# lightkurve/lightkurve

Measured on AMD Instinct MI355X. Metric: frequencies*targets/sec (Lomb-Scargle, ls_method='fast' (reference default): extirpolation + FFT) + BLS periods*targets/sec; max-power rel-err, higher is better.
Workload: dtype f64

## Files before the change

lightkurve_amd/csrc/lsfast.hip:

```cpp
#include <cmath>
#include <cstdlib>
#include <type_traits>
#include <vector>

#include "lk_common.hpp"
#include "ls_epilogue.hpp"

namespace lk {

typedef double lk_d2v __attribute__((ext_vector_type(2)));

constexpr int SPREAD_W = 1024;
constexpr int SPREAD_WW = 256;

struct FastStats {
    double wsum, ybar, YY, t0;
    double yws;
    double wmax;
    double vmax;
};

__device__ __forceinline__ void cadence_weights(const double *__restrict__ y, const double *__restrict__ dy, int64_t i,
                                                double wsum, double ybar, double &w, double &wy) {
    const double d = dy ? dy[i] : 1.0;
// ... 77 lines not shown
        }
        yws = bsum(acc2);
        wmx = bmax(wmx);
        vmx = bmax(vmx);
    }
    if (tid == 0) stats[b] = FastStats{wsum, ybar, YY, t0, yws, wmx, vmx};
}

constexpr int TAB_PER_LANE = 8;
__global__ __launch_bounds__(256) void lsf_tables_kernel(const double *__restrict__ t, const int64_t *__restrict__ n_off,
                                                          const FastStats *__restrict__ stats,
                                                          const int *__restrict__ rows_used, double df, int nfft, int m2,
                                                          int logW, int *__restrict__ spread_tab, int ntab) {
    const int b = blockIdx.y;
    if (!rows_used[b * 4 + 3]) return;
    const int64_t lo = n_off[b], n = n_off[b + 1] - lo;
    const int lane = threadIdx.x & 63;
    const int64_t base = ((int64_t)blockIdx.x * 4 + (threadIdx.x >> 6)) * (64 * TAB_PER_LANE);
    if (base >= n) return;
    const double t0 = stats[b].t0;
    int *tab = spread_tab + (size_t)b * 4 * ntab;
    const double iW = 1.0 / (double)(1 << logW), dn = (double)nfft;
    auto posn = [&](double tt) {
        const double x = (tt - t0) * dn * df;
        return x < dn ? x : fmod(x, dn);
    };
    double p1[TAB_PER_LANE];
#pragma unroll
    for (int u = 0; u < TAB_PER_LANE; ++u) {
        const int64_t i = base + 64 * u + lane;
        p1[u] = posn(t[lo + (i < n ? i : n - 1)]);
    }
    const int nf0 = min(ntab, (int)((((long long)rows_used[b * 4 + 0] << m2) >> logW) + 3));
    const int nf2 = min(ntab, (int)((((long long)rows_used[b * 4 + 2] << m2) >> logW) + 3));
    double prev_last = base > 0 ? posn(t[lo + base - 1]) : -1e300;
#pragma unroll
    for (int u = 0; u < TAB_PER_LANE; ++u) {
        const int64_t i = base + 64 * u + lane;
        double pp1 = __shfl_up(p1[u], 1);
        if (lane == 0) pp1 = prev_last;
        prev_last = __shfl(p1[u], 63);
        if (i >= n) continue;
#pragma unroll
        for (int gg = 0; gg < 2; ++gg) {
            const double p = gg ? 2.0 * p1[u] : p1[u], pp = i > 0 ? (gg ? 2.0 * pp1 : pp1) : -1e300;
            int *lo_a = tab + (size_t)(2 * gg) * ntab, *hi_a = lo_a + ntab;
            const int nfill = gg ? nf2 : nf0;
            int k0 = i > 0 ? (int)floor((pp + 4.0) * iW) + 1 : 0, k1 = (int)floor((p + 4.0) * iW);
            for (int k = max(k0, 0); k <= min(k1, ntab - 1); ++k) lo_a[k] = (int)i;
            if (i == n - 1)
                for (int k = max(k1 + 1, 0); k < nfill; ++k) lo_a[k] = (int)n;
            k0 = i > 0 ? (int)floor((pp - 3.0) * iW) + 1 : 0;
            k1 = (int)floor((p - 3.0) * iW);
            for (int k = max(k0, 0); k <= min(k1, ntab - 1); ++k) hi_a[k] = (int)i;
            if (i == n - 1)
                for (int k = max(k1 + 1, 0); k < nfill; ++k) hi_a[k] = (int)n;
        }
    }
}

__device__ __forceinline__ void phase_factor(double f, double tt, double &c, double &s) {
    const double p = f * tt, e = fma(f, tt, -p);
    const double r = (p - rint(p)) + e;
    sincospi(2.0 * r, &s, &c);
}

struct Stencil4 {
    int i0, n;
    double wt[4];
};
__device__ __forceinline__ Stencil4 stencil4(double x, int nfft) {
    Stencil4 st;
    if (x == floor(x)) {
        st.i0 = (int)x;
        st.n = 1;
        st.wt[0] = 1.0;
        st.wt[1] = st.wt[2] = st.wt[3] = 0.0;
        return st;
    }
    int ilo = (int)(x - 2.0);
    ilo = min(max(ilo, 0), nfft - 4);
    const double d0 = x - (double)ilo, d1 = d0 - 1.0, d2 = d0 - 2.0, d3 = d0 - 3.0;
    st.i0 = ilo;
    st.n = 4;
    st.wt[3] = ((d0 * d1) * d2) * (1.0 / 6.0);
    st.wt[2] = ((d0 * d1) * d3) * -0.5;
    st.wt[1] = ((d0 * d2) * d3) * 0.5;
    st.wt[0] = ((d1 * d2) * d3) * (-1.0 / 6.0);
    return st;
}

struct Quantum {
    double q, iq;
    __device__ __forceinline__ void add(double *cell, double v) const {
        if (q > 0.0)
            atomicAdd(reinterpret_cast<unsigned long long *>(cell), (unsigned long long)(long long)rint(v * iq));
        else
            unsafeAtomicAdd(cell, v);
    }
};
__device__ __forceinline__ Quantum make_quantum(double vmax) {
    const double q = (vmax > 0.0 && isfinite(vmax)) ? ldexp(1.0, ilogb(1.25 * vmax) - 49) : 0.0;
    return Quantum{q, q > 0.0 ? 1.0 / q : 0.0};
}

__device__ __forceinline__ void extirpolate4(double2 *__restrict__ grid, const Stencil4 &sp, double hr, double hi,
                                             const Quantum &Q) {
#pragma unroll
    for (int k = 0; k < 4; ++k)
        if (k < sp.n) {
            Q.add(&grid[sp.i0 + k].x, hr * sp.wt[k]);
            Q.add(&grid[sp.i0 + k].y, hi * sp.wt[k]);
        }
}

__global__ __launch_bounds__(256) void lsf_scatter_kernel(const double *__restrict__ t, const double *__restrict__ y,
                                                           const double *__restrict__ dy,
                                                           const int64_t *__restrict__ n_off,
                                                           const FastStats *__restrict__ stats, int b0, double f0,
                                                           double df, int nfft, int fit_mean,
                                                           double2 *__restrict__ grids,
                                                           const int *__restrict__ rows_used) {
    if (rows_used && rows_used[blockIdx.y * 4 + 3]) return;
    const int b = b0 + blockIdx.y;
    const int64_t lo = n_off[b];
    const int n = (int)(n_off[b + 1] - lo);
    const int i = blockIdx.x * 256 + threadIdx.x;
    if (i >= n) return;
    const FastStats st = stats[b];
    const double tt = t[lo + i] - st.t0;
    double2 *g0 = grids + (size_t)blockIdx.y * 3 * nfft, *g1 = g0 + nfft, *g2 = g1 + nfft;
    double wi, wyi;
    cadence_weights(y, dy, lo + i, st.wsum, st.ybar, wi, wyi);
    const Quantum Qy = make_quantum(st.vmax), Qw = make_quantum(st.wmax);
    for (int fac = 1; fac <= 2; ++fac) {
        const double dff = df * (double)fac, f0f = f0 * (double)fac;
        double c = 1.0, s = 0.0;
        if (f0f > 0.0) phase_factor(f0f, tt, c, s);
        const Stencil4 sp = stencil4(fmod(tt * (double)nfft * dff, (double)nfft), nfft);
        if (fac == 1) {
            extirpolate4(g0, sp, wyi * c, wyi * s, Qy);
            if (fit_mean) extirpolate4(g1, sp, wi * c, wi * s, Qw);
        } else {
            extirpolate4(g2, sp, wi * c, wi * s, Qw);
        }
    }
}

__global__ __launch_bounds__(256) void lsf_spread_owner_kernel(const double *__restrict__ t, const double *__restrict__ y,
                                                                const double *__restrict__ dy,
                                                                const int64_t *__restrict__ n_off,
                                                                const FastStats *__restrict__ stats, int b0, double f0,
                                                                double df, int nfft, int m2, int fit_mean,
                                                                double2 *__restrict__ grids,
                                                                const int *__restrict__ rows_used,
                                                                const int *__restrict__ spread_tab, int ntab) {
    __shared__ double2 acc0[SPREAD_W], acc1[SPREAD_W];
    const int lb = blockIdx.y, tid = threadIdx.x;
    const bool pair = blockIdx.z == 0;
    if (!rows_used[lb * 4 + 3]) return;
    const int g = pair ? 0 : 2;
    const int ncell = rows_used[lb * 4 + g] << m2;
    const int c_lo = blockIdx.x * SPREAD_W, c_hi = min(c_lo + SPREAD_W, ncell);
    if (c_lo >= ncell) return;
    double2 *G0 = grids + ((size_t)lb * 3 + g) * (size_t)nfft, *G1 = G0 + nfft;
    const int b = b0 + lb;
    const int64_t lo = n_off[b];
    const FastStats st = stats[b];
    const double fac = pair ? 1.0 : 2.0;
    const double dff = df * fac, f0f = f0 * fac;
    for (int c = tid; c < SPREAD_W; c += 256) {
        acc0[c] = make_double2(0.0, 0.0);
        acc1[c] = make_double2(0.0, 0.0);
    }
    __syncthreads();
    const int lane = tid & 63, wv = tid >> 6;
    const int w_lo = c_lo + wv * SPREAD_WW, w_hi = min(w_lo + SPREAD_WW, c_hi);
    if (w_lo < w_hi) {
        const int *tab = spread_tab + ((size_t)b * 4 + (pair ? 0 : 2)) * ntab;
        const int kblk = blockIdx.x * (SPREAD_W / SPREAD_WW) + wv;
        const int i_lo = tab[kblk], i_hi = tab[ntab + min(kblk + 1, ntab - 1)];
        for (int i = i_lo + lane; i < i_hi; i += 64) {
            const double tt = t[lo + i] - st.t0;
            double wi, wyi;
            cadence_weights(y, dy, lo + i, st.wsum, st.ybar, wi, wyi);
            double c = 1.0, s = 0.0;
            if (f0f > 0.0) phase_factor(f0f, tt, c, s);
            const Stencil4 sp = stencil4(fmod(tt * (double)nfft * dff, (double)nfft), nfft);
            const double ar = (pair ? wyi : wi) * c, ai = (pair ? wyi : wi) * s, br = wi * c, bi = wi * s;
#pragma unroll
            for (int k = 0; k < 4; ++k) {
                const int cell = sp.i0 + k;
                if (k < sp.n && cell >= w_lo && cell < w_hi) {
                    unsafeAtomicAdd(&acc0[cell - c_lo].x, ar * sp.wt[k]);
                    unsafeAtomicAdd(&acc0[cell - c_lo].y, ai * sp.wt[k]);
                    if (pair && fit_mean) {
                        unsafeAtomicAdd(&acc1[cell - c_lo].x, br * sp.wt[k]);
                        unsafeAtomicAdd(&acc1[cell - c_lo].y, bi * sp.wt[k]);
                    }
                }
            }
        }
    }
    __syncthreads();
    for (int c = c_lo + tid; c < c_hi; c += 256) {
        G0[c] = acc0[c - c_lo];
        if (pair) G1[c] = acc1[c - c_lo];
    }
}

__device__ __forceinline__ void lds_fft_dit(double2 *x, const double2 *tw, int n, int m, int nf) {
    const int tid = threadIdx.x, nt = blockDim.x;
    const int halfn = n >> 1;
    for (int s = 1; s <= m; ++s) {
        const int half = 1 << (s - 1);
        const int tstep = n >> s;
        for (int p = tid; p < nf * halfn; p += nt) {
            const int f = p >> (m - 1), j = p & (halfn - 1);
            const int grp = j >> (s - 1), k = j & (half - 1);
            const int i0 = f * n + (grp << s) + k, i1 = i0 + half;
            const double2 wv = tw[k * tstep];
            const double2 a = x[i0], bq = x[i1];
            const double tr = wv.x * bq.x - wv.y * bq.y, ti = wv.x * bq.y + wv.y * bq.x;
            x[i0] = make_double2(a.x + tr, a.y + ti);
            x[i1] = make_double2(a.x - tr, a.y - ti);
        }
        __syncthreads();
    }
}

__device__ __forceinline__ void lds_twiddles(double2 *tw, int n) {
    for (int k = threadIdx.x; k < (n >> 1); k += blockDim.x) {
        double s, c;
        sincospi(2.0 * (double)k / (double)n, &s, &c);
        tw[k] = make_double2(c, s);
    }
}

__global__ __launch_bounds__(256) void fft_cols_kernel(double2 *__restrict__ grids, int m1, int m2, int CT) {
    extern __shared__ __attribute__((aligned(16))) double2 lds2[];
    const int N1 = 1 << m1, N2 = 1 << m2;
    double2 *x = lds2, *tw = lds2 + (size_t)CT * N1;
    double2 *G = grids + ((size_t)blockIdx.y << (m1 + m2));
    const int c0 = blockIdx.x * CT;
    lds_twiddles(tw, N1);
    for (int e = threadIdx.x; e < CT * N1; e += 256) {
        const int r = e / CT, cc = e - r * CT;
        const int rr = (int)(__brev((unsigned)r) >> (32 - m1));
        x[cc * N1 + rr] = G[(size_t)r * N2 + c0 + cc];
    }
    __syncthreads();
    lds_fft_dit(x, tw, N1, m1, CT);
    const double invN = 1.0 / (double)((size_t)1 << (m1 + m2));
    for (int e = threadIdx.x; e < CT * N1; e += 256) {
        const int k1 = e / CT, cc = e - k1 * CT;
        const long long ck = (long long)(c0 + cc) * k1;
        double s, c;
        sincospi(2.0 * (double)ck * invN, &s, &c);
        const double2 v = x[cc * N1 + k1];
        G[(size_t)k1 * N2 + c0 + cc] = make_double2(v.x * c - v.y * s, v.x * s + v.y * c);
    }
}

__global__ __launch_bounds__(256) void fft_rows_kernel(const double2 *__restrict__ grids, int m1, int m2, int RT,
                                                        int nkeep, double2 *__restrict__ spec) {
    extern __shared__ __attribute__((aligned(16))) double2 lds2[];
    const int N2 = 1 << m2;
    double2 *x = lds2, *tw = lds2 + (size_t)RT * N2;
    const double2 *G = grids + ((size_t)blockIdx.y << (m1 + m2));
    double2 *S = spec + (size_t)blockIdx.y * nkeep;
    const int r0 = blockIdx.x * RT;
    lds_twiddles(tw, N2);
    for (int e = threadIdx.x; e < RT * N2; e += 256) {
        const int rr = e / N2, c = e - rr * N2;
        const int cr = m2 ? (int)(__brev((unsigned)c) >> (32 - m2)) : 0;
        x[rr * N2 + cr] = G[(size_t)(r0 + rr) * N2 + c];
    }
    __syncthreads();
    lds_fft_dit(x, tw, N2, m2, RT);
    for (int e = threadIdx.x; e < RT * N2; e += 256) {
        const int k2 = e / RT, rr = e - k2 * RT;
        const long long k = (long long)(r0 + rr) + ((long long)k2 << m1);
        if (k < nkeep) S[k] = x[rr * N2 + k2];
    }
}

__device__ constexpr double R32C[16] = {1.0, 0.98078528040323043, 0.92387953251128674, 0.83146961230254524,
                                        0.70710678118654752, 0.55557023301960218, 0.38268343236508978,
                                        0.19509032201612825, 0.0, -0.19509032201612825, -0.38268343236508978,
                                        -0.55557023301960218, -0.70710678118654752, -0.83146961230254524,
                                        -0.92387953251128674, -0.98078528040323043};
__device__ constexpr double R32S[16] = {0.0, 0.19509032201612825, 0.38268343236508978, 0.55557023301960218,
                                        0.70710678118654752, 0.83146961230254524, 0.92387953251128674,
                                        0.98078528040323043, 1.0, 0.98078528040323043, 0.92387953251128674,
                                        0.83146961230254524, 0.70710678118654752, 0.55557023301960218,
                                        0.38268343236508978, 0.19509032201612825};

__host__ __device__ constexpr int brev_c(int x, int bits) {
    int r = 0;
    for (int i = 0; i < bits; ++i) r |= ((x >> i) & 1) << (bits - 1 - i);
    return r;
}

template <int L>
__device__ __forceinline__ void reg_fft(double2 (&v)[1 << L]) {
#pragma unroll
    for (int s = L; s >= 1; --s) {
        const int half = 1 << (s - 1);
#pragma unroll
        for (int g = 0; g < (1 << L); g += (1 << s)) {
#pragma unroll
            for (int k = 0; k < half; ++k) {
                const double2 a = v[g + k], b = v[g + k + half];
                v[g + k] = make_double2(a.x + b.x, a.y + b.y);
                const double dx = a.x - b.x, dy = a.y - b.y;
                const int ti = k * (32 >> s);
                if (ti == 0)
                    v[g + k + half] = make_double2(dx, dy);
                else if (ti == 8)
                    v[g + k + half] = make_double2(-dy, dx);
                else
                    v[g + k + half] = make_double2(dx * R32C[ti] - dy * R32S[ti], dx * R32S[ti] + dy * R32C[ti]);
            }
        }
    }
}

__device__ __forceinline__ double2 cmul(double2 a, double2 b) {
    return make_double2(a.x * b.x - a.y * b.y, a.x * b.y + a.y * b.x);
}

template <int LA, int LB, int MODE, class Load, class Store>
__device__ __forceinline__ void block_fft(int NF, double2 *tile, Load load, Store store, int tw = 1) {
    constexpr int A = 1 << LA, Bq = 1 << LB, n = A * Bq, LDT = Bq + 1, FST = A * LDT + 1;
    const int tid = threadIdx.x;
    if (tid < NF * Bq) {
        int f, j;
        if (MODE == 1) {
            f = tid % NF;
            j = tid / NF;
        } else if (MODE == 2) {
            const int jl = tid % tw, rest = tid / tw;
            f = rest % NF;
            j = jl + tw * (rest / NF);
        } else {
            f = tid / Bq;
            j = tid % Bq;
        }
        double2 v[A];
#pragma unroll
        for (int i = 0; i < A; ++i) v[i] = load(f, i * Bq + j);
        reg_fft<LA>(v);
        double s1, c1;
        sincospi(2.0 * (double)j / (double)n, &s1, &c1);
        const double2 step = make_double2(c1, s1);
        double2 w = make_double2(1.0, 0.0);
        double2 *row = tile + (size_t)f * FST + j;
#pragma unroll
        for (int ka = 0; ka < A; ++ka) {
            row[ka * LDT] = cmul(v[brev_c(ka, LA)], w);
            w = cmul(w, step);
        }
    }
    __syncthreads();
    if (tid < NF * A) {
        const int ka = tid / NF, f = tid - ka * NF;
        const double2 *row = tile + (size_t)f * FST + (size_t)ka * LDT;
        double2 u[Bq];
#pragma unroll
        for (int j = 0; j < Bq; ++j) u[j] = row[j];
        reg_fft<LB>(u);
#pragma unroll
        for (int kb = 0; kb < Bq; ++kb) store(f, ka + A * kb, u[brev_c(kb, LB)], kb);
    }
}

template <int LA, int LB>
__global__ __launch_bounds__(256) void fft_cols_reg_kernel(double2 *__restrict__ grids, int m2, int CT,
                                                            const int *__restrict__ rows_used,
                                                            double2 *__restrict__ gout, int tw) {
    extern __shared__ __attribute__((aligned(16))) double2 lds2[];
    constexpr int m1 = LA + LB, A = 1 << LA;
    const int N2 = 1 << m2;
    double2 *G = grids + ((size_t)blockIdx.y << (m1 + m2));
    const int c0 = blockIdx.x * CT;
    const int ru = rows_used ? rows_used[(blockIdx.y / 3) * 4 + (blockIdx.y % 3)] : (1 << m1);
    const double invN = 1.0 / (double)((size_t)1 << (m1 + m2));
    auto load = [&](int f, int r) -> double2 {
        return r < ru ? G[(size_t)r * N2 + c0 + f] : make_double2(0.0, 0.0);
    };
    int last_f = -1;
    double2 w = make_double2(1.0, 0.0), step = w;
    const int twl = 31 - __clz(max(tw, 1));
    auto store = [&](int f, int k1, double2 v, int) {
        const int c = c0 + f;
        if (f != last_f) {
            double s, cc;
            sincospi(2.0 * (double)((long long)c * k1) * invN, &s, &cc);
            w = make_double2(cc, s);
            sincospi(2.0 * (double)((long long)c * A) * invN, &s, &cc);
            step = make_double2(cc, s);
            last_f = f;
        }
        if (gout)
            gout[((size_t)blockIdx.y << (m1 + m2)) + ((((size_t)(c >> twl) << m1) + k1) << twl) + (c & (tw - 1))] = cmul(v, w);
        else
            G[(size_t)k1 * N2 + c] = cmul(v, w);
        w = cmul(w, step);
    };
    block_fft<LA, LB, 1>(CT, lds2, load, store);
}

constexpr int PRUNED_CT = 16;

constexpr int LSF_CHUNK_HALF_GB = 3;

template <int LP>
__global__ __launch_bounds__(PRUNED_CT * (1 << ((LP + 1) / 2)), 2) void fft_cols_pruned_kernel(
    const double2 *__restrict__ grids, int m1, int m2, const int *__restrict__ rows_used, double2 *__restrict__ gout,
    const double *__restrict__ t, const double *__restrict__ y, const double *__restrict__ dy,
    const int64_t *__restrict__ n_off, const FastStats *__restrict__ stats, int b0, double f0, double df, int fit_mean,
    const int *__restrict__ tab16, int ntab16) {
    extern __shared__ __attribute__((aligned(16))) double2 lds2[];
    constexpr int LA = (LP + 1) / 2, LB = LP / 2, A = 1 << LA, Bq = 1 << LB, P = 1 << LP, LDT = Bq + 1, FST = A * LDT + 1;
    constexpr int CT = PRUNED_CT, NT = CT * A;
    const int N1 = 1 << m1, N2 = 1 << m2, Q = N1 >> LP;
    const double2 *G = grids + ((size_t)blockIdx.y << (m1 + m2));
    const size_t tstride = (size_t)CT << m1, gstride = (size_t)(N2 / CT) * tstride;
    double2 *O = gout + (size_t)blockIdx.y * gstride + (size_t)blockIdx.x * tstride;
    const int c0 = blockIdx.x * CT;
    const int lbt = blockIdx.y / 3, g = blockIdx.y % 3;
    const int ru = rows_used[lbt * 4 + g];
    const int tid = threadIdx.x;
    const int f = tid % CT, jk = tid / CT;
    const bool p1 = jk < Bq, p2 = jk < A;
    const double invN1 = 1.0 / (double)N1, invN = 1.0 / (double)((size_t)1 << (m1 + m2));
    double2 xin[A];
    if (tab16 != nullptr && rows_used[lbt * 4 + 3]) {
        double2 *acc = lds2;
        for (int e = tid; e < ru * CT; e += NT) acc[e] = make_double2(0.0, 0.0);
        __syncthreads();
        if (!(g == 1 && !fit_mean)) {
            const int b = b0 + lbt;
            const int64_t lo = n_off[b];
            const FastStats st = stats[b];
            const double fac = g == 2 ? 2.0 : 1.0, dff = df * fac, f0f = f0 * fac, dn = (double)((size_t)1 << (m1 + m2));
            const int nfft = 1 << (m1 + m2);
            const int *tlo = tab16 + ((size_t)b * 4 + (g == 2 ? 2 : 0)) * ntab16, *thi = tlo + ntab16;
            const int S = g == 2 ? 4 : 8, rpi = 64 / S;
            const int lane = tid & 63, wv = tid >> 6, rr = lane / S, k = lane - rr * S;
            const int rpw = (ru + NT / 64 - 1) / (NT / 64);
            const int r_end = min(ru, (wv + 1) * rpw);
            auto visit = [&](int r, double ti, double yi, double di) {
                const double tt = ti - st.t0;
                const double wi = (1.0 / (di * di)) / st.wsum, wyi = wi * (yi - st.ybar);
                double c = 1.0, sn = 0.0;
                if (f0f > 0.0) phase_factor(f0f, tt, c, sn);
                const double xp = tt * dn * dff;
                const Stencil4 sp = stencil4(xp < dn ? xp : fmod(xp, dn), nfft);
                const double amp = g == 0 ? wyi : wi, ar = amp * c, ai = amp * sn;
                const int cbase = (r << m2) + c0;
#pragma unroll
                for (int q = 0; q < 4; ++q) {
                    const unsigned col = (unsigned)(sp.i0 + q - cbase);
                    if (q < sp.n && col < (unsigned)CT) {
                        unsafeAtomicAdd(&acc[r * CT + col].x, ar * sp.wt[q]);
                        unsafeAtomicAdd(&acc[r * CT + col].y, ai * sp.wt[q]);
                    }
                }
            };
            constexpr int UN = 4;
            for (int rb = wv * rpw; rb < r_end; rb += UN * rpi) {
                int ii[UN], ih[UN];
#pragma unroll
                for (int u = 0; u < UN; ++u) {
                    const int r = rb + u * rpi + rr;
                    const int blk = (min(r, r_end - 1) << (m2 - 4)) + blockIdx.x;
                    ii[u] = tlo[blk] + k;
                    ih[u] = thi[blk + 1];
                }
#pragma unroll
                for (int u = 0; u < UN; ++u) {
                    asm volatile("" : "+v"(ii[u]), "+v"(ih[u]));
                    if (rb + u * rpi + rr >= r_end) ii[u] = ih[u] = 0;
                }
                double tv[UN], yv[UN], dv[UN];
#pragma unroll
                for (int u = 0; u < UN; ++u) {
                    const bool ok = ii[u] < ih[u];
                    const int64_t ix = lo + (ok ? ii[u] : 0);
                    tv[u] = t[ix];
                    yv[u] = y[ix];
                    dv[u] = dy ? dy[ix] : 1.0;
                }
#pragma unroll
                for (int u = 0; u < UN; ++u) {
                    const int r = rb + u * rpi + rr;
                    if (ii[u] < ih[u]) visit(r, tv[u], yv[u], dv[u]);
                    int i = ii[u] + S;
                    while (__any(i < ih[u])) {
                        if (i < ih[u]) visit(r, t[lo + i], y[lo + i], dy ? dy[lo + i] : 1.0);
                        i += S;
                    }
                }
            }
        }
        __syncthreads();
        if (p1) {
#pragma unroll
            for (int i = 0; i < A; ++i) {
                const int r = i * Bq + jk;
                xin[i] = r < ru ? acc[r * CT + f] : make_double2(0.0, 0.0);
            }
        }
        __syncthreads();
    } else if (p1) {
#pragma unroll
        for (int i = 0; i < A; ++i) {
            const int r = i * Bq + jk;
            xin[i] = r < ru ? G[(size_t)r * N2 + c0 + f] : make_double2(0.0, 0.0);
        }
    }
    auto root = [](double x) {
        double sn, cs;
        sincospi(2.0 * x, &sn, &cs);
        return make_double2(cs, sn);
    };
    const double2 wj = root((double)jk * invN1), wq = root((double)Bq * invN1);
    const double2 tw_j = root((double)jk / (double)P);
    const double2 wc = root((double)(c0 + f) * invN), stepc = root((double)((long long)(c0 + f) * Q * A) * invN);
    double2 wjs = make_double2(1.0, 0.0), wqs = wjs;
    double2 wout = root((double)((long long)(c0 + f) * Q * jk) * invN);
    for (int s = 0; s < Q; ++s) {
        if (p1) {
            double2 v[A];
            if (s == 0) {
#pragma unroll
                for (int i = 0; i < A; ++i) v[i] = xin[i];
            } else {
                double2 w = wjs;
#pragma unroll
                for (int i = 0; i < A; ++i) {
                    v[i] = cmul(xin[i], w);
                    w = cmul(w, wqs);
                }
            }
            reg_fft<LA>(v);
            double2 w = make_double2(1.0, 0.0);
            double2 *row = lds2 + (size_t)f * FST + jk;
#pragma unroll
            for (int ka = 0; ka < A; ++ka) {
                row[ka * LDT] = cmul(v[brev_c(ka, LA)], w);
                w = cmul(w, tw_j);
            }
        }
        __syncthreads();
        if (p2) {
            const double2 *row = lds2 + (size_t)f * FST + (size_t)jk * LDT;
            double2 u[Bq];
#pragma unroll
            for (int j = 0; j < Bq; ++j) u[j] = row[j];
            reg_fft<LB>(u);
            double2 w = wout;
#pragma unroll
            for (int kb = 0; kb < Bq; ++kb) {
                const int q = jk + A * kb;
                O[(size_t)(Q * q + s) * CT + f] = cmul(u[brev_c(kb, LB)], w);
                w = cmul(w, stepc);
            }
        }
        wjs = cmul(wjs, wj);
        wqs = cmul(wqs, wq);
        wout = cmul(wout, wc);
        __syncthreads();
    }
}

template <int LA, int LB>
__global__ __launch_bounds__(256) void fft_rows_reg_kernel(const double2 *__restrict__ grids, int m1, int RT, int nkeep,
                                                            double2 *__restrict__ spec) {
    extern __shared__ __attribute__((aligned(16))) double2 lds2[];
    constexpr int m2 = LA + LB;
    const int N2 = 1 << m2;
    const double2 *G = grids + ((size_t)blockIdx.y << (m1 + m2));
    double2 *S = spec + (size_t)blockIdx.y * nkeep;
    const int r0 = blockIdx.x * RT;
    auto load = [&](int f, int c) -> double2 { return G[(size_t)(r0 + f) * N2 + c]; };
    auto store = [&](int f, int k2, double2 v, int) {
        const long long k = (long long)(r0 + f) + ((long long)k2 << m1);
        if (k < nkeep) S[k] = v;
    };
    block_fft<LA, LB, 0>(RT, lds2, load, store);
}

struct PeakPart {
    double v;
    long long k;
};

__device__ __forceinline__ bool peak_better(double v2, long long k2, double v, long long k) {
    return k2 >= 0 && (k < 0 || v2 > v || (v2 == v && k2 < k));
}

template <int LA, int LB, int KB>
__global__ __launch_bounds__(512) void fft_rows_power_kernel(const double2 *__restrict__ grids, int m1, int RT,
                                                              const int64_t *__restrict__ n_off,
                                                              const FastStats *__restrict__ stats, int b0, double f0,
                                                              double df, int64_t M, int fit_mean, int norm,
                                                              const double *__restrict__ scale,
                                                              double *__restrict__ power, int tw,
                                                              PeakPart *__restrict__ peaks) {
    extern __shared__ __attribute__((aligned(16))) double2 lds2[];
    constexpr int m2 = LA + LB, A = 1 << LA;
    const int N2 = 1 << m2;
    const int twl = tw ? 31 - __clz(tw) : 0;
    const size_t tstride = tw ? ((size_t)tw << m1) : 0, gstride = (size_t)1 << (m1 + m2);
    const int lb = blockIdx.y, r0 = blockIdx.x * RT;
    double2 keep0[KB], keep1[KB], keep2[KB];
#pragma unroll
    for (int q = 0; q < KB; ++q) keep0[q] = keep1[q] = keep2[q] = make_double2(0.0, 0.0);
    auto transform = [&](int g, double2(&keep)[KB]) {
        const double2 *G = grids + (size_t)(lb * 3 + g) * gstride;
        auto load = [&](int f, int c) -> double2 {
            return tw ? G[(size_t)(c >> twl) * tstride + ((size_t)(r0 + f) << twl) + (c & (tw - 1))] : G[(size_t)(r0 + f) * N2 + c];
        };
        auto store = [&](int, int, double2 v, int kb) {
            if (kb < KB) keep[kb < KB ? kb : 0] = v;
        };
        if (tw)
            block_fft<LA, LB, 2>(RT, lds2, load, store, tw);
        else
            block_fft<LA, LB, 0>(RT, lds2, load, store);
    };
    transform(0, keep0);
    __syncthreads();
    if (fit_mean) transform(1, keep1);
    __syncthreads();
    transform(2, keep2);
    const int tid = threadIdx.x;
    double best_v = 0.0;
    long long best_k = -1;
    if (tid < RT * A) {
        const int ka = tid / RT, f = tid - ka * RT;
        const int b = b0 + lb;
        const FastStats st = stats[b];
        const double nn = (double)(n_off[b + 1] - n_off[b]);
        const double sc = scale ? scale[b] : 1.0;
        const int k1 = r0 + f;
        const double twopi = 6.283185307179586;
        double ph_c = 1.0, ph_s = 0.0, st_c = 1.0, st_s = 0.0;
        if (st.t0 != 0.0) {
            const long long kfirst = (long long)k1 + ((long long)ka << m1);
            sincos(twopi * st.t0 * (f0 + df * (double)kfirst), &ph_s, &ph_c);
            sincos(twopi * st.t0 * (df * (double)((long long)A << m1)), &st_s, &st_c);
        }
#pragma unroll
        for (int kb = 0; kb < KB; ++kb) {
            const long long k = (long long)k1 + ((long long)(ka + A * kb) << m1);
            if (k < M) {
                double2 a = keep0[kb], bq = keep1[kb], c2 = keep2[kb];
                if (st.t0 != 0.0) {
                    const double c = ph_c, s = ph_s;
                    a = make_double2(a.x * c - a.y * s, a.x * s + a.y * c);
                    bq = make_double2(bq.x * c - bq.y * s, bq.x * s + bq.y * c);
                    const double cc = c * c - s * s, ss = 2.0 * s * c;
                    c2 = make_double2(c2.x * cc - c2.y * ss, c2.x * ss + c2.y * cc);
                }
                const double pw = gls_power_sums(a.y, a.x, bq.y, bq.x, c2.y, c2.x, fit_mean, norm, st.YY, 0.5 * st.wsum, nn, sc);
                power[(size_t)b * (size_t)M + k] = pw;
                if (pw == pw && peak_better(pw, k, best_v, best_k)) {
                    best_v = pw;
                    best_k = k;
                }
            }
            const double nc = ph_c * st_c - ph_s * st_s, ns = ph_s * st_c + ph_c * st_s;
            ph_c = nc;
            ph_s = ns;
        }
    }
    if (peaks == nullptr) return;
#pragma unroll
    for (int o = 32; o > 0; o >>= 1) {
        const double v2 = __shfl_xor(best_v, o);
        const long long k2 = __shfl_xor(best_k, o);
        if (peak_better(v2, k2, best_v, best_k)) {
            best_v = v2;
            best_k = k2;
        }
    }
    if ((tid & 63) == 0)
        peaks[((size_t)lb * gridDim.x + blockIdx.x) * (blockDim.x >> 6) + (tid >> 6)] = PeakPart{best_v, best_k};
}

__device__ __forceinline__ double dpp_ror8(double x) {
    int lo = __double2loint(x), hi = __double2hiint(x);
    lo = __builtin_amdgcn_update_dpp(0, lo, 0x128, 0xF, 0xF, true);
    hi = __builtin_amdgcn_update_dpp(0, hi, 0x128, 0xF, 0xF, true);
    return __hiloint2double(hi, lo);
}

struct Rows512 {
    static constexpr int RT = 8;
    static constexpr int SK = 34;
    static constexpr int SF = 16 * SK + 4;
    static constexpr int NT = RT * 32;
    static constexpr size_t LDS_BYTES = (size_t)RT * SF * 8;
};

__global__ __launch_bounds__(Rows512::NT, 2) void fft_rows512_power_kernel(
    const double2 *__restrict__ grids, int m1, int ntargets, const int64_t *__restrict__ n_off,
    const FastStats *__restrict__ stats, int b0, double f0, double df, int64_t M, int fit_mean, int norm,
    const double *__restrict__ scale, double *__restrict__ power, PeakPart *__restrict__ peaks) {
    using R = Rows512;
    constexpr int RT = R::RT, SK = R::SK, SF = R::SF;
    extern __shared__ __attribute__((aligned(16))) double tile512[];
    const int tid = threadIdx.x;
    const size_t gstride = (size_t)1 << (m1 + 9);
    const int tiles_per_target = (1 << m1) / RT;
    const int jl = tid & 15, f1 = (tid >> 4) & (RT - 1), jh = tid >> 7, j = jl + 16 * jh;
    const int f2 = tid & 7, e = (tid >> 3) & 1, ka = tid >> 4;
    auto tile_base = [&](int T) {
        const int lbT = ntargets - 1 - T / tiles_per_target, r0T = (T % tiles_per_target) * RT;
        return grids + (size_t)lbT * 3 * gstride + ((size_t)jh << (m1 + 4)) + ((size_t)(r0T + f1) << 4) + jl;
    };
    double2 v[16];
    auto load = [&](const double2 *G) {
#pragma unroll
        for (int i = 0; i < 16; ++i) {
            const lk_d2v q = __builtin_nontemporal_load(reinterpret_cast<const lk_d2v *>(G + ((size_t)i << (m1 + 5))));
            v[i] = make_double2(q.x, q.y);
        }
    };
    double2 step1, step4;
    {
        double s, c;
        sincospi((double)j * (1.0 / 256.0), &s, &c);
        step1 = make_double2(c, s);
        sincospi((double)j * (1.0 / 64.0), &s, &c);
        step4 = make_double2(c, s);
    }
    double2 keep[3][4];
    double *row1 = tile512 + f1 * SF + j;
    const double *row2 = tile512 + f2 * SF + ka * SK + e;
    auto process = [&](auto Gc, auto refill) {
        constexpr int G = decltype(Gc)::value;
        __builtin_amdgcn_sched_barrier(0);
        reg_fft<4>(v);
        __builtin_amdgcn_sched_barrier(0);
        {
            double2 w = step1;
#pragma unroll
            for (int bb = 1; bb < 4; ++bb) {
#pragma unroll
                for (int a = 0; a < 4; ++a) v[brev_c(4 * a + bb, 4)] = cmul(v[brev_c(4 * a + bb, 4)], w);
                if (bb < 3) w = cmul(w, step1);
            }
        }
        __builtin_amdgcn_sched_barrier(0);
        {
            double2 w = step4;
#pragma unroll
            for (int a = 1; a < 4; ++a) {
#pragma unroll
                for (int bb = 0; bb < 4; ++bb) v[brev_c(4 * a + bb, 4)] = cmul(v[brev_c(4 * a + bb, 4)], w);
                if (a < 3) w = cmul(w, step4);
            }
        }
        __builtin_amdgcn_sched_barrier(0);
        double ure[16], uim[16];
#pragma unroll
        for (int k = 0; k < 16; ++k) row1[k * SK] = v[brev_c(k, 4)].x;
        __syncthreads();
#pragma unroll
        for (int jj = 0; jj < 16; ++jj) ure[jj] = row2[2 * jj];
        __syncthreads();
#pragma unroll
        for (int k = 0; k < 16; ++k) row1[k * SK] = v[brev_c(k, 4)].y;
        __builtin_amdgcn_sched_barrier(0);
        refill();
        __syncthreads();
#pragma unroll
        for (int jj = 0; jj < 16; ++jj) uim[jj] = row2[2 * jj];
        __builtin_amdgcn_sched_barrier(0);
        double2 s0[8], s1[8];
#pragma unroll
        for (int q = 0; q < 8; ++q) {
            s0[q] = make_double2(ure[2 * q], uim[2 * q]);
            s1[q] = make_double2(ure[2 * q + 1], uim[2 * q + 1]);
        }
        reg_fft<3>(s0);
        __builtin_amdgcn_sched_barrier(0);
        reg_fft<3>(s1);
        __builtin_amdgcn_sched_barrier(0);
        auto pval = [&](int kb) -> double2 {
            const double2 a = s0[brev_c(kb, 3)], bq = s1[brev_c(kb, 3)];
            double2 hsum;
            if (kb == 0)
                hsum = make_double2(a.x + bq.x, a.y + bq.y);
            else if (kb == 4)
                hsum = make_double2(a.x - bq.y, a.y + bq.x);
            else
                hsum = make_double2(a.x + (bq.x * R32C[2 * kb] - bq.y * R32S[2 * kb]),
                                    a.y + (bq.x * R32S[2 * kb] + bq.y * R32C[2 * kb]));
            if (kb == 0) return hsum;
            const double wc = e ? R32C[kb] : 1.0, ws = e ? R32S[kb] : 0.0;
            return make_double2(hsum.x * wc - hsum.y * ws, hsum.x * ws + hsum.y * wc);
        };
#pragma unroll
        for (int q = 0; q < 4; ++q) {
            const double2 plo = pval(q), phi = pval(q + 4);
            const double2 mine = e ? phi : plo, send = e ? plo : phi;
            keep[G][q] = make_double2(mine.x + dpp_ror8(send.x), mine.y + dpp_ror8(send.y));
            __builtin_amdgcn_sched_barrier(0);
        }
    };
    using I0 = std::integral_constant<int, 0>;
    using I1 = std::integral_constant<int, 1>;
    using I2 = std::integral_constant<int, 2>;
    const int T = blockIdx.x;
    const double2 *Gt = tile_base(T);
    load(Gt);
    {
        const int lb = ntargets - 1 - T / tiles_per_target, r0 = (T % tiles_per_target) * RT;
        process(I0{}, [&] { load(Gt + gstride); });
        __syncthreads();
        process(I1{}, [&] { load(Gt + 2 * gstride); });
        __syncthreads();
        process(I2{}, [] {});
        double best_v = 0.0;
        long long best_k = -1;
        {
            const int b = b0 + lb;
            const FastStats st = stats[b];
            const double nn = (double)(n_off[b + 1] - n_off[b]);
            const double sc = scale ? scale[b] : 1.0;
            const int k1 = r0 + f2;
            const double twopi = 6.283185307179586;
            double ph_c = 1.0, ph_s = 0.0, st_c = 1.0, st_s = 0.0;
            if (st.t0 != 0.0) {
                const long long kfirst = (long long)k1 + ((long long)(ka + 64 * e) << m1);
                sincos(twopi * st.t0 * (f0 + df * (double)kfirst), &ph_s, &ph_c);
                sincos(twopi * st.t0 * (df * (double)((long long)16 << m1)), &st_s, &st_c);
            }
#pragma unroll 1
            for (int q = 0; q < 4; ++q) {
                const long long k = (long long)k1 + ((long long)(ka + 16 * (4 * e + q)) << m1);
                if (k < M) {
                    double2 a = keep[0][0], bq = keep[1][0], c2 = keep[2][0];
                    if (st.t0 != 0.0) {
                        const double c = ph_c, s = ph_s;
                        a = make_double2(a.x * c - a.y * s, a.x * s + a.y * c);
                        bq = make_double2(bq.x * c - bq.y * s, bq.x * s + bq.y * c);
                        const double cc = c * c - s * s, ss = 2.0 * s * c;
                        c2 = make_double2(c2.x * cc - c2.y * ss, c2.x * ss + c2.y * cc);
                    }
                    const double pw = gls_power_sums(a.y, a.x, bq.y, bq.x, c2.y, c2.x, fit_mean, norm, st.YY, 0.5 * st.wsum, nn, sc);
                    power[(size_t)b * (size_t)M + k] = pw;
                    if (pw == pw && peak_better(pw, k, best_v, best_k)) {
                        best_v = pw;
                        best_k = k;
                    }
                }
                const double nc = ph_c * st_c - ph_s * st_s, ns = ph_s * st_c + ph_c * st_s;
                ph_c = nc;
                ph_s = ns;
#pragma unroll
                for (int g = 0; g < 3; ++g)
#pragma unroll
                    for (int r = 0; r < 3; ++r) keep[g][r] = keep[g][r + 1];
            }
        }
        if (peaks != nullptr) {
#pragma unroll
            for (int o = 32; o > 0; o >>= 1) {
                const double v2 = __shfl_xor(best_v, o);
                const long long k2 = __shfl_xor(best_k, o);
                if (peak_better(v2, k2, best_v, best_k)) {
                    best_v = v2;
                    best_k = k2;
                }
            }
            if ((tid & 63) == 0)
                peaks[((size_t)lb * tiles_per_target + (T % tiles_per_target)) * (R::NT / 64) + (tid >> 6)] = PeakPart{best_v, best_k};
        }
    }
}

__global__ __launch_bounds__(64) void lsf_peaks_kernel(const PeakPart *__restrict__ peaks, int nparts, int b0,
                                                        double *__restrict__ max_out, int64_t *__restrict__ arg_out) {
    const PeakPart *pp = peaks + (size_t)blockIdx.x * nparts;
    double v = 0.0;
    long long k = -1;
    for (int i = threadIdx.x; i < nparts; i += 64)
        if (peak_better(pp[i].v, pp[i].k, v, k)) {
            v = pp[i].v;
            k = pp[i].k;
        }
#pragma unroll
    for (int o = 32; o > 0; o >>= 1) {
        const double v2 = __shfl_xor(v, o);
        const long long k2 = __shfl_xor(k, o);
        if (peak_better(v2, k2, v, k)) {
            v = v2;
            k = k2;
        }
    }
    if (threadIdx.x == 0) {
        max_out[b0 + blockIdx.x] = k >= 0 ? v : NAN;
        arg_out[b0 + blockIdx.x] = (int64_t)k;
    }
}

__global__ __launch_bounds__(256) void lsf_scatter_multi_kernel(const double *__restrict__ t, const double *__restrict__ y,
                                                                 const double *__restrict__ dy,
                                                                 const int64_t *__restrict__ n_off,
                                                                 const FastStats *__restrict__ stats, int b0, double f0,
                                                                 double df, int nfft, int nterms,
                                                                 double2 *__restrict__ grids) {
    const int b = b0 + blockIdx.y;
    const int64_t lo = n_off[b];
    const int n = (int)(n_off[b + 1] - lo);
    const int i = blockIdx.x * 256 + threadIdx.x;
    if (i >= n) return;
    const FastStats st = stats[b];
    const double tt = t[lo + i] - st.t0;
    double2 *g0 = grids + (size_t)blockIdx.y * 3 * nterms * nfft;
    double wi, wyi;
    cadence_weights(y, dy, lo + i, st.wsum, st.ybar, wi, wyi);
    const Quantum Qy = make_quantum(st.vmax), Qw = make_quantum(st.wmax);
    for (int fac = 1; fac <= 2 * nterms; ++fac) {
        const double dff = df * (double)fac, f0f = f0 * (double)fac;
        double c = 1.0, s = 0.0;
        if (f0f > 0.0) phase_factor(f0f, tt, c, s);
        const Stencil4 sp = stencil4(fmod(tt * (double)nfft * dff, (double)nfft), nfft);
        extirpolate4(g0 + (size_t)(nterms + fac - 1) * nfft, sp, wi * c, wi * s, Qw);
        if (fac <= nterms) extirpolate4(g0 + (size_t)(fac - 1) * nfft, sp, wyi * c, wyi * s, Qy);
    }
}

template <int NT>
__global__ __launch_bounds__(256) void lsf_chi2_power_kernel(const double2 *__restrict__ spec,
                                                              const int64_t *__restrict__ n_off,
                                                              const FastStats *__restrict__ stats, int b0, double f0,
                                                              double df, int64_t M, int fit_mean, int norm,
                                                              const double *__restrict__ scale,
                                                              double *__restrict__ power) {
    const int b = b0 + blockIdx.y;
    const int64_t j = (int64_t)blockIdx.x * 256 + threadIdx.x;
    if (j >= M) return;
    const FastStats st = stats[b];
    const double2 *s0 = spec + (size_t)blockIdx.y * 3 * NT * M;
    Chi2Sums<NT> sums;
    const double twopi = 6.283185307179586;
#pragma unroll
    for (int m = 1; m <= 2 * NT; ++m) {
        double cph = 1.0, sph = 0.0;
        if (st.t0 != 0.0) sincos(twopi * st.t0 * (double)m * (f0 + df * (double)j), &sph, &cph);
        const double2 a = s0[(size_t)(NT + m - 1) * M + j];
        sums.Cw[m - 1] = a.x * cph - a.y * sph;
        sums.Sw[m - 1] = a.x * sph + a.y * cph;
        if (m <= NT) {
            const double2 y = s0[(size_t)(m - 1) * M + j];
            sums.Cy[m - 1] = y.x * cph - y.y * sph;
            sums.Sy[m - 1] = y.x * sph + y.y * cph;
        }
    }
    const double n = (double)(n_off[b + 1] - n_off[b]);
    power[(size_t)b * (size_t)M + j] =
        chi2_normalise(sums.solve_lu(st.yws, fit_mean), norm, st.YY, 0.5 * st.wsum, n, scale ? scale[b] : 1.0);
}

__global__ __launch_bounds__(256) void lsf_power_kernel(const double2 *__restrict__ spec,
                                                         const int64_t *__restrict__ n_off,
                                                         const FastStats *__restrict__ stats, int b0, double f0,
                                                         double df, int64_t M, int fit_mean, int norm,
                                                         const double *__restrict__ scale,
                                                         double *__restrict__ power) {
    const int b = b0 + blockIdx.y;
    const int64_t j = (int64_t)blockIdx.x * 256 + threadIdx.x;
    if (j >= M) return;
    const FastStats st = stats[b];
    const double2 *s0 = spec + (size_t)blockIdx.y * 3 * M;
    double2 a = s0[j], bq = s0[M + j], c2 = s0[2 * M + j];
    if (st.t0 != 0.0) {
        const double twopi = 6.283185307179586;
        double s, c;
        sincos(twopi * st.t0 * (f0 + df * (double)j), &s, &c);
        a = make_double2(a.x * c - a.y * s, a.x * s + a.y * c);
        bq = make_double2(bq.x * c - bq.y * s, bq.x * s + bq.y * c);
        sincos(twopi * st.t0 * (2.0 * f0 + 2.0 * df * (double)j), &s, &c);
        c2 = make_double2(c2.x * c - c2.y * s, c2.x * s + c2.y * c);
    }
    const double n = (double)(n_off[b + 1] - n_off[b]);
    power[(size_t)b * (size_t)M + j] = gls_power_sums(a.y, a.x, bq.y, bq.x, c2.y, c2.x, fit_mean, norm, st.YY,
                                                      0.5 * st.wsum, n, scale ? scale[b] : 1.0);
}

__global__ __launch_bounds__(256) void lsf_unquantize_kernel(double2 *__restrict__ grids, int m1, int m2,
                                                              const int *__restrict__ rows_used,
                                                              const FastStats *__restrict__ stats, int b0, int ngp, int n_wy) {
    const int lbt = blockIdx.y / ngp, g = blockIdx.y % ngp;
    if (rows_used && rows_used[lbt * 4 + 3]) return;
    const int ru = rows_used ? rows_used[lbt * 4 + g] : (1 << m1);
    const FastStats st = stats[b0 + lbt];
    const double q = make_quantum(g < n_wy ? st.vmax : st.wmax).q;
    if (!(q > 0.0)) return;
    const int N2 = 1 << m2;
    double2 *G = grids + ((size_t)blockIdx.y << (m1 + m2));
    for (int r = blockIdx.x * 8; r < min(blockIdx.x * 8 + 8, ru); ++r)
        for (int c = threadIdx.x; c < N2; c += 256) {
            const double2 v = G[(size_t)r * N2 + c];
            G[(size_t)r * N2 + c] = make_double2((double)__double_as_longlong(v.x) * q, (double)__double_as_longlong(v.y) * q);
        }
}

__global__ __launch_bounds__(256) void lsf_zero_kernel(double2 *__restrict__ grids, int m1, int m2,
                                                        const int *__restrict__ rows_used) {
    if (rows_used[(blockIdx.y / 3) * 4 + 3]) return;
    const int ru = rows_used[(blockIdx.y / 3) * 4 + (blockIdx.y % 3)];
    const int N2 = 1 << m2;
    double2 *G = grids + ((size_t)blockIdx.y << (m1 + m2));
    for (int r = blockIdx.x * 8; r < min(blockIdx.x * 8 + 8, ru); ++r)
        for (int c = threadIdx.x; c < N2; c += 256) G[(size_t)r * N2 + c] = make_double2(0.0, 0.0);
}

constexpr int COLS_TILE_PTS = 4096;

template <int LA, int LB>
static void launch_cols_t(lk_handle *h, int m2, int ngrids, double2 *grids, const int *rows_used, double2 *gout, int tw,
                          hipStream_t stream) {
    constexpr int A = 1 << LA, Bq = 1 << LB, n = A * Bq, LDT = Bq + 1, FST = A * LDT + 1;
    const int N2 = 1 << m2;
    const int CT = std::max(1, std::min(N2, std::min(COLS_TILE_PTS / n, 256 / std::max(A, Bq))));
    const int nt = ((CT * std::max(A, Bq) + 63) / 64) * 64;
    (void)want_lds(h, reinterpret_cast<const void *>(fft_cols_reg_kernel<LA, LB>), 160 * 1024);
    hipLaunchKernelGGL((fft_cols_reg_kernel<LA, LB>), dim3(N2 / CT, ngrids), dim3(nt), (size_t)CT * FST * 16, stream, grids,
                       m2, CT, rows_used, gout, tw);
}

static int tile_width(int m1, int m2) {
    const int la1 = (m1 + 1) / 2, lb1 = m1 / 2, n1 = 1 << m1;
    const int ct = std::max(1, std::min(1 << m2, std::min(COLS_TILE_PTS / n1, 256 / std::max(1 << la1, 1 << lb1))));
    const int bq2 = 1 << (m2 / 2);
    return std::min(ct, bq2);
}

template <int LA, int LB>
static void launch_rows_t(lk_handle *h, int m1, int ngrids, const double2 *grids, int nkeep, double2 *spec, hipStream_t stream) {
    constexpr int A = 1 << LA, Bq = 1 << LB, n = A * Bq, LDT = Bq + 1, FST = A * LDT + 1;
    const int N1 = 1 << m1;
    const int RT = std::max(1, std::min(N1, std::min(4096 / n, 256 / std::max(A, Bq))));
    const int nt = ((RT * std::max(A, Bq) + 63) / 64) * 64;
    (void)want_lds(h, reinterpret_cast<const void *>(fft_rows_reg_kernel<LA, LB>), 100 * 1024);
    hipLaunchKernelGGL((fft_rows_reg_kernel<LA, LB>), dim3(N1 / RT, ngrids), dim3(nt), (size_t)RT * FST * 16, stream,
                       grids, m1, RT, nkeep, spec);
}

struct FusedArgs {
    const int64_t *n_off;
    const FastStats *stats;
    int b0;
    double f0, df;
    int64_t M;
    int fit_mean, norm;
    const double *scale;
    double *power;
    PeakPart *peaks;
};

template <int LA, int LB>
static int rows_power_rt(int m1) {
    constexpr int A = 1 << LA, Bq = 1 << LB, n = A * Bq;
    return std::max(1, std::min(1 << m1, std::min(4096 / n, 256 / std::max(A, Bq))));
}

template <int LA, int LB, int KB>
static void launch_rows_power_t(lk_handle *h, int m1, int ntargets, const double2 *grids, const FusedArgs &a, int tw,
                                hipStream_t stream) {
    constexpr int A = 1 << LA, Bq = 1 << LB, LDT = Bq + 1, FST = A * LDT + 1;
    const int N1 = 1 << m1;
    const int RT = rows_power_rt<LA, LB>(m1);
    const int nt = ((RT * std::max(A, Bq) + 63) / 64) * 64;
    (void)want_lds(h, reinterpret_cast<const void *>(fft_rows_power_kernel<LA, LB, KB>), 160 * 1024);
    hipLaunchKernelGGL((fft_rows_power_kernel<LA, LB, KB>), dim3(N1 / RT, ntargets), dim3(nt), (size_t)RT * FST * 16,
                       stream, grids, m1, RT, a.n_off, a.stats, a.b0, a.f0, a.df, a.M, a.fit_mean, a.norm, a.scale,
                       a.power, tw, a.peaks);
}

static bool rows_power_available(int m1, int m2, int64_t M) {
    const int LA = (m2 + 1) / 2, Aa = 1 << LA;
    const long long k2need = (M + ((long long)1 << m1) - 1) >> m1;
    return m2 >= 4 && m2 <= 10 && (k2need + Aa - 1) / Aa <= 8;
}

#define LK_M2_SWITCH(m2, X) \
    switch (m2) {           \
        case 4: X(2, 2)     \
        case 5: X(3, 2)     \
        case 6: X(3, 3)     \
        case 7: X(4, 3)     \
        case 8: X(4, 4)     \
        case 9: X(5, 4)     \
        default: X(5, 5)    \
    }

static int rows_power_parts(int m1, int m2) {
#define LK_X(la, lb)                                                                                   \
    {                                                                                                  \
        const int rt = rows_power_rt<la, lb>(m1);                                                      \
        return ((1 << m1) / rt) * ((rt * std::max(1 << (la), 1 << (lb)) + 63) / 64);                   \
    }
    LK_M2_SWITCH(m2, LK_X)
#undef LK_X
}

static bool rows512_applies(int m1, int m2, int64_t M, int tw) {
    const long long k2need = (M + ((long long)1 << m1) - 1) >> m1;
    return m2 == 9 && tw == PRUNED_CT && m1 >= 3 && k2need <= 128;
}

static void launch_rows512(lk_handle *h, int m1, int ntargets, const double2 *grids, const FusedArgs &a, hipStream_t stream) {
    const int ntiles = ((1 << m1) / Rows512::RT) * ntargets;
    hipLaunchKernelGGL(fft_rows512_power_kernel, dim3(ntiles), dim3(Rows512::NT), Rows512::LDS_BYTES, stream, grids, m1, ntargets,
                       a.n_off, a.stats, a.b0, a.f0, a.df, a.M, a.fit_mean, a.norm, a.scale, a.power, a.peaks);
}

static bool launch_rows_power(lk_handle *h, int m1, int m2, int ntargets, const double2 *grids, const FusedArgs &a, int tw,
                              hipStream_t stream) {
    const int LA = (m2 + 1) / 2, Aa = 1 << LA;
    const long long k2need = (a.M + ((long long)1 << m1) - 1) >> m1;
    if (rows512_applies(m1, m2, a.M, tw)) {
        launch_rows512(h, m1, ntargets, grids, a, stream);
        return true;
    }
    const int kb = (int)((k2need + Aa - 1) / Aa);
    if (kb > 8 || m2 < 4 || m2 > 10) return false;
#define LK_X(la, lb)                                                            \
    {                                                                           \
        if (kb <= 4)                                                            \
            launch_rows_power_t<la, lb, 4>(h, m1, ntargets, grids, a, tw, stream); \
        else                                                                    \
            launch_rows_power_t<la, lb, 8>(h, m1, ntargets, grids, a, tw, stream); \
        return true;                                                            \
    }
    LK_M2_SWITCH(m2, LK_X)
#undef LK_X
}

static void launch_cols_reg(lk_handle *h, int m1, int m2, int ngrids, double2 *grids, const int *rows_used, double2 *gout,
// ... 327 lines not shown
```

Baseline: 9.484 billion.

## Skip zero-padded FFT inputs and unneeded output quarters in Lomb-Scargle FFT

Adds a compile-time variant of the register FFT that treats the upper half of its inputs as zero, and uses it when the used rows fit in half the pass size. This halves the input twiddle multiplies and skips the first butterfly stage for short inputs. In the final kernel, the output quarters are reassigned so each lane pair handles interleaved frequency blocks, and work for quarters past the needed frequency count M is skipped via a wave-uniform count. The phase-start and step for the t0 correction are adjusted to match the new ordering. Correctness depends on the reindexing being consistent with the stores.

```diff
diff --git a/lightkurve_amd/csrc/lsfast.hip b/lightkurve_amd/csrc/lsfast.hip
--- a/lightkurve_amd/csrc/lsfast.hip
+++ b/lightkurve_amd/csrc/lsfast.hip
@@ -403,7 +403,7 @@
     return r;
 }
 
-template <int L>
+template <int L, bool UPPER_ZERO = false>
 __device__ __forceinline__ void reg_fft(double2 (&v)[1 << L]) {
 #pragma unroll
     for (int s = L; s >= 1; --s) {
@@ -412,9 +412,10 @@
         for (int g = 0; g < (1 << L); g += (1 << s)) {
 #pragma unroll
             for (int k = 0; k < half; ++k) {
-                const double2 a = v[g + k], b = v[g + k + half];
-                v[g + k] = make_double2(a.x + b.x, a.y + b.y);
-                const double dx = a.x - b.x, dy = a.y - b.y;
+                const bool bz = UPPER_ZERO && s == L;
+                const double2 a = v[g + k], b = bz ? make_double2(0.0, 0.0) : v[g + k + half];
+                if (!bz) v[g + k] = make_double2(a.x + b.x, a.y + b.y);
+                const double dx = bz ? a.x : a.x - b.x, dy = bz ? a.y : a.y - b.y;
                 const int ti = k * (32 >> s);
                 if (ti == 0)
                     v[g + k + half] = make_double2(dx, dy);
@@ -536,6 +537,7 @@
     const int f = tid % CT, jk = tid / CT;
     const bool p1 = jk < Bq, p2 = jk < A;
     const double invN1 = 1.0 / (double)N1, invN = 1.0 / (double)((size_t)1 << (m1 + m2));
+    const bool short_in = ru <= P / 2;
     double2 xin[A];
     if (tab16 != nullptr && rows_used[lbt * 4 + 3]) {
         double2 *acc = lds2;
@@ -632,49 +634,57 @@
     const double2 wc = root((double)(c0 + f) * invN), stepc = root((double)((long long)(c0 + f) * Q * A) * invN);
     double2 wjs = make_double2(1.0, 0.0), wqs = wjs;
     double2 wout = root((double)((long long)(c0 + f) * Q * jk) * invN);
-    for (int s = 0; s < Q; ++s) {
-        if (p1) {
-            double2 v[A];
-            if (s == 0) {
-#pragma unroll
-                for (int i = 0; i < A; ++i) v[i] = xin[i];
-            } else {
-                double2 w = wjs;
-#pragma unroll
-                for (int i = 0; i < A; ++i) {
-                    v[i] = cmul(xin[i], w);
-                    w = cmul(w, wqs);
+    auto passes = [&](auto short_c) {
+        constexpr bool SHORT = decltype(short_c)::value;
+        constexpr int AI = SHORT ? A / 2 : A;
+        for (int s = 0; s < Q; ++s) {
+            if (p1) {
+                double2 v[A];
+                if (s == 0) {
+#pragma unroll
+                    for (int i = 0; i < AI; ++i) v[i] = xin[i];
+                } else {
+                    double2 w = wjs;
+#pragma unroll
+                    for (int i = 0; i < AI; ++i) {
+                        v[i] = cmul(xin[i], w);
+                        if (i + 1 < AI) w = cmul(w, wqs);
+                    }
+                }
+                reg_fft<LA, SHORT>(v);
+                double2 w = make_double2(1.0, 0.0);
+                double2 *row = lds2 + (size_t)f * FST + jk;
+#pragma unroll
+                for (int ka = 0; ka < A; ++ka) {
+                    row[ka * LDT] = cmul(v[brev_c(ka, LA)], w);
+                    w = cmul(w, tw_j);
                 }
             }
-            reg_fft<LA>(v);
-            double2 w = make_double2(1.0, 0.0);
-            double2 *row = lds2 + (size_t)f * FST + jk;
-#pragma unroll
-            for (int ka = 0; ka < A; ++ka) {
-                row[ka * LDT] = cmul(v[brev_c(ka, LA)], w);
-                w = cmul(w, tw_j);
+            __syncthreads();
+            if (p2) {
+                const double2 *row = lds2 + (size_t)f * FST + (size_t)jk * LDT;
+                double2 u[Bq];
+#pragma unroll
+                for (int j = 0; j < Bq; ++j) u[j] = row[j];
+                reg_fft<LB>(u);
+                double2 w = wout;
+#pragma unroll
+                for (int kb = 0; kb < Bq; ++kb) {
+                    const int q = jk + A * kb;
+                    O[(size_t)(Q * q + s) * CT + f] = cmul(u[brev_c(kb, LB)], w);
+                    w = cmul(w, stepc);
+                }
             }
-        }
-        __syncthreads();
-        if (p2) {
-            const double2 *row = lds2 + (size_t)f * FST + (size_t)jk * LDT;
-            double2 u[Bq];
-#pragma unroll
-            for (int j = 0; j < Bq; ++j) u[j] = row[j];
-            reg_fft<LB>(u);
-            double2 w = wout;
-#pragma unroll
-            for (int kb = 0; kb < Bq; ++kb) {
-                const int q = jk + A * kb;
-                O[(size_t)(Q * q + s) * CT + f] = cmul(u[brev_c(kb, LB)], w);
-                w = cmul(w, stepc);
-            }
-        }
-        wjs = cmul(wjs, wj);
-        wqs = cmul(wqs, wq);
-        wout = cmul(wout, wc);
-        __syncthreads();
-    }
+            wjs = cmul(wjs, wj);
+            wqs = cmul(wqs, wq);
+            wout = cmul(wout, wc);
+            __syncthreads();
+        }
+    };
+    if (short_in)
+        passes(std::true_type{});
+    else
+        passes(std::false_type{});
 }
 
 template <int LA, int LB>
@@ -841,6 +851,8 @@
         step4 = make_double2(c, s);
     }
     double2 keep[3][4];
+    const int k2need = (int)((M + ((int64_t)1 << m1) - 1) >> m1);
+    const int nq = __builtin_amdgcn_readfirstlane(min(4, (k2need - 4 * (tid >> 6) + 31) >> 5));
     double *row1 = tile512 + f1 * SF + j;
     const double *row2 = tile512 + f2 * SF + ka * SK + e;
     auto process = [&](auto Gc, auto refill) {
@@ -909,9 +921,11 @@
         };
 #pragma unroll
         for (int q = 0; q < 4; ++q) {
-            const double2 plo = pval(q), phi = pval(q + 4);
-            const double2 mine = e ? phi : plo, send = e ? plo : phi;
-            keep[G][q] = make_double2(mine.x + dpp_ror8(send.x), mine.y + dpp_ror8(send.y));
+            if (q < nq) {
+                const double2 pev = pval(2 * q), pod = pval(2 * q + 1);
+                const double2 mine = e ? pod : pev, send = e ? pev : pod;
+                keep[G][q] = make_double2(mine.x + dpp_ror8(send.x), mine.y + dpp_ror8(send.y));
+            }
             __builtin_amdgcn_sched_barrier(0);
         }
     };
@@ -939,13 +953,13 @@
             const double twopi = 6.283185307179586;
             double ph_c = 1.0, ph_s = 0.0, st_c = 1.0, st_s = 0.0;
             if (st.t0 != 0.0) {
-                const long long kfirst = (long long)k1 + ((long long)(ka + 64 * e) << m1);
+                const long long kfirst = (long long)k1 + ((long long)(ka + 16 * e) << m1);
                 sincos(twopi * st.t0 * (f0 + df * (double)kfirst), &ph_s, &ph_c);
-                sincos(twopi * st.t0 * (df * (double)((long long)16 << m1)), &st_s, &st_c);
+                sincos(twopi * st.t0 * (df * (double)((long long)32 << m1)), &st_s, &st_c);
             }
 #pragma unroll 1
-            for (int q = 0; q < 4; ++q) {
-                const long long k = (long long)k1 + ((long long)(ka + 16 * (4 * e + q)) << m1);
+            for (int q = 0; q < nq; ++q) {
+                const long long k = (long long)k1 + ((long long)(ka + 16 * (2 * q + e)) << m1);
                 if (k < M) {
                     double2 a = keep[0][0], bq = keep[1][0], c2 = keep[2][0];
                     if (st.t0 != 0.0) {
```

After: 9.825 billion, median of 6. +3.6%, better.
